# Roco-scientist/NGS-Barcode-Count

Hardware: AMD Instinct MI355X
Metric: reads/sec (whole node), 3x8nt DEL vs 3x1k refs (higher is better)
Workload: dtype u8

## Files before the change

ngs-barcode-count_amd/csrc/bc_device_plan.h:

```cpp
#pragma once
#include "bc_intrin.h"

#ifdef BC_JIT_TU
extern "C" __constant__ uint64_t bc_jit_addr[];
#define BC_ADDR(field, k) bc_jit_addr[index * kAddrPerGroup + (k)]
#define BC_PLAN_ADDR(field, k) bc_jit_addr[kMaxGroups * kAddrPerGroup + (k)]
#define BC_ADDR_COLD(field, k) (*reinterpret_cast<const volatile uint64_t*>(&bc_jit_addr[index * kAddrPerGroup + (k)]))
#else
#define BC_ADDR_COLD(field, k) field
#define BC_ADDR(field, k) field
#define BC_PLAN_ADDR(field, k) field
#endif

namespace bc {

constexpr int kMaxGroups = 18;
constexpr int kAddrPerGroup = 17;
constexpr int kPlanAddrs = 1;
constexpr int kMaxEntries = 160;
constexpr int kMaxRuns = 40;
constexpr int kClasses = 5;
constexpr int kMaxNW = 10;
constexpr uint32_t kFail = 0xFFFFFFFFu;
constexpr uint32_t kDeferred = 0xFFFFFFFEu;
// ... 134 lines not shown
BC_HD uint64_t wide_fingerprint(const uint64_t* key, uint32_t W) {
  uint64_t h = 0x9E3779B97F4A7C15ull;
#pragma unroll
  for (uint32_t w = 1; w < (uint32_t)kMaxKeyWords; ++w)
    if (w < W) h = wide_mix(h ^ key[w]) + w;
  return h >> 1;
}
BC_HD void wide_or_bits(uint64_t (&key)[kMaxKeyWords], uint32_t at, uint32_t v, uint32_t n) {
  const uint32_t w0 = 1u + (at >> 6), sh = at & 63u;
  const uint64_t x = (uint64_t)(v & lowmask(n));
  const bool spill = sh + n > 64u;
  const uint64_t lo = x << sh, hi = spill ? x >> ((64u - sh) & 63u) : 0ull;
#pragma unroll
  for (uint32_t w = 1; w < (uint32_t)kMaxKeyWords; ++w) {
    if (w == w0) key[w] |= lo;
    if (w == w0 + 1u) key[w] |= hi;
  }
}
BC_HD void wide_or_planes(uint64_t (&key)[kMaxKeyWords], uint32_t at, uint32_t q1, uint32_t q2, uint32_t qn, uint32_t len) {
  wide_or_bits(key, at, q1 & ~qn, len);
  wide_or_bits(key, at + len, q2 & ~qn, len);
  wide_or_bits(key, at + 2u * len, qn, len);
}

constexpr int kNCounters = 8;
constexpr int kTotalReads = 6;

enum Outcome : uint32_t {
  kMatched = 0, kConstantRegion = 1, kSampleBarcode = 2, kBarcode = 3, kDuplicate = 4, kLowQuality = 5,
  kPending = 6,
  kUnsupported = 7
};

}
```

ngs-barcode-count_amd/csrc/bc_engine.hip:

```cpp
#include <hip/hip_runtime.h>
#include <string.h>
#include <stdio.h>
#include <stdlib.h>
#include <unistd.h>

#include <algorithm>
#include <functional>
#include <thread>
#include <unordered_map>
#include <string>
#include <vector>

#include "../../include/barcode_count_hip.h"
#include "bc_kernel.h"
#include "bc_engine_impl.h"
#include "bc_fold.h"
#include "bc_synth.h"

extern "C" int bc_internal_table_pack_u8(const void* d_table_u32, const void* d_bits, uint64_t n, void* d_out_u8, void* d_ovf_idx_u64,
                                         void* d_ovf_val_u32, uint64_t ovf_capacity, uint64_t* n_ovf, int device_id, void* hip_stream);

namespace bc {

template <int NW, int NWW>
// ... 614 lines not shown
      if (G.seed_nb) {
        if ((rc = upload(e, H.seed_off.data(), H.seed_off.size() * 4, &G.seed_off_a))) return rc;
        if ((rc = upload(e, H.seed_list.data(), H.seed_list.size() * 4, &G.seed_list_a))) return rc;
        if ((rc = upload(e, H.odd_list.data(), H.odd_list.size() * 4, &G.odd_list_a))) return rc;
        if (G.seed2_nb) {
          if ((rc = upload(e, H.seed2_off.data(), H.seed2_off.size() * 4, &G.seed2_off_a))) return rc;
          if ((rc = upload(e, H.seed2_list.data(), H.seed2_list.size() * 4, &G.seed2_list_a))) return rc;
        }
        if (G.seed3_nb) {
          if ((rc = upload(e, H.seed3_off.data(), H.seed3_off.size() * 4, &G.seed3_off_a))) return rc;
          if ((rc = upload(e, H.seed3_list.data(), H.seed3_list.size() * 4, &G.seed3_list_a))) return rc;
        }
        if (G.tier_blen) {
          if ((rc = upload(e, H.tier_off.data(), H.tier_off.size() * 4, &G.tier_off_a))) return rc;
          if ((rc = upload(e, H.tier_list.data(), H.tier_list.size() * 4, &G.tier_list_a))) return rc;
          if ((rc = upload(e, H.tier_bkt.data(), H.tier_bkt.size() * 4, &G.tier_bkt_a))) return rc;
        }
      }
    }
    if (G.mode == kSetDirect) {
      void* d = nullptr;
      HIP_TRY(hipMalloc(&d, (size_t)4 << (2 * G.len)));
      e->allocs.push_back(d);
      G.dtable_a = (uint64_t)(uintptr_t)d;
    }
  }
  if (const char* cl = getenv("BC_COUNT_LOG")) e->count_log = strcmp(cl, "auto") == 0 ? 2 : atoi(cl);
  if (const char* ch = getenv("BC_COUNT_LOG_HOT")) e->log_hot = atoi(ch) != 0;
  if (const char* cd = getenv("BC_COUNT_LOG_DEFER_RESET")) e->defer_reset = atoi(cd) != 0;
  if (const char* cf = getenv("BC_COUNT_LOG_FRESH")) e->fold_fresh = atoi(cf) != 0;
  if (const char* cm = getenv("BC_COUNT_LOG_MIN_READS")) e->log_min_reads = strtoull(cm, nullptr, 0);
  if (const char* cc = getenv("BC_COUNT_LOG_CHUNK")) {
    const uint64_t c = strtoull(cc, nullptr, 0) & ~63ull;
    if (c) e->log_chunk = std::min<uint64_t>(c, 1ull << 27);
  }
  if (P.lhash_vec) {
    const int rc = upload(e, e->h.lhash.data(), e->h.lhash.size() * 4, &P.lhash_a);
    if (rc) return rc;
  }
#ifdef BC_EXPERIMENT
  if (const char* pm = getenv("BC_PIPE")) e->pipe = atoi(pm) != 0;
#endif
  e->qshare = qual_region_shared();
  HIP_TRY(hipMalloc((void**)&e->d_plan, sizeof(DevPlan)));
  HIP_TRY(hipMemcpy(e->d_plan, &P, sizeof(DevPlan), hipMemcpyHostToDevice));
  for (uint32_t g = 0; g < P.n_groups; ++g) {
    const DevGroup& G = P.groups[g];
    if (G.mode != kSetDirect) continue;
    const uint32_t nq = 1u << (2 * G.len);
    hipLaunchKernelGGL(build_dtable_kernel, dim3((nq + 255) / 256), dim3(256), 0, e->stream, e->d_plan, g,
                       reinterpret_cast<uint32_t*>((uintptr_t)G.dtable_a));
    HIP_TRY(hipGetLastError());
  }
  if (P.sparse) {
    if (table_mem) {
      set_error("bc_engine_create: the plan keeps raw captures (no dense table); pass table_mem = NULL");
      return BC_ERR_INVALID;
    }
  } else if (table_mem) {
    e->d_table = (uint32_t*)table_mem;
    e->table_all_dirty = true;
  } else {
    HIP_TRY(hipMalloc((void**)&e->d_table, e->table_entries * 4));
    e->own_table = true;
    HIP_TRY(hipMemsetAsync(e->d_table, 0, e->table_entries * 4, e->stream));
  }
  if (e->n_bit_words) {
// ... 157 lines not shown
  const OwedPlan owed = owed_plan(e, use_log, table_untouched);
  if (owed.table == kOwedMain) {
    const int rc = settle_table_on(e, e->stream);
    if (rc != BC_OK) return rc;
  }
  if (owed.bits == kOwedMain) {
    const int rc = settle_bits_on(e, e->stream);
    if (rc != BC_OK) return rc;
  }
  const uint32_t flags = (s.pipe ? 1u : 0u) | (s.tables_generic ? 2u : 0u) | (s.hot_generic && hot_on ? 4u : 0u);
  if (s.lds + 64 > e->lds_limit) {
    set_error("read stride too large for one LDS tile");
    return BC_ERR_UNSUPPORTED;
  }
  const bool wide = e->h.plan.wide != 0;
  const void* kern = wide ? (const void*)match_count_wide_kernel<NW, NWW> : (const void*)match_count_kernel<NW, NWW>;
  if (s.lds > 48 * 1024) HIP_TRY(hipFuncSetAttribute(kern, hipFuncAttributeMaxDynamicSharedMemorySize, (int)s.lds));
  int per_cu = 0;
  HIP_TRY(hipOccupancyMaxActiveBlocksPerMultiprocessor(&per_cu, kern, kTPB, lds));
  if (per_cu < 1) per_cu = 1;
  const uint64_t resident = (uint64_t)per_cu * e->n_cus;
  const uint64_t blocks = std::min<uint64_t>((n_reads + kTPB - 1) / kTPB, resident);
  uint64_t blocks_jit = blocks, resident_jit = resident;
  hipEvent_t e0 = nullptr, e1 = nullptr;
  if (e->timing) {
    HIP_TRY(hipEventCreate(&e0));
    HIP_TRY(hipEventCreate(&e1));
    HIP_TRY(hipEventRecord(e0, e->stream));
  }
  hipFunction_t jit_fn = nullptr;
  e->reads_seen += n_reads;
  if (NW <= 8 && NWW <= 4 && e->jit_mode != 0) {
    int per_cu_jit = 1;
    jit_fn = e->jit.function(e->h.plan, e->device, e->jit_mode, e->reads_seen, s, hot_on, &per_cu_jit);
    resident_jit = (uint64_t)per_cu_jit * e->n_cus;
    if (jit_fn) blocks_jit = std::min<uint64_t>((n_reads + kTPB - 1) / kTPB, resident_jit);
  }
  if (use_log) {
    const int rc = ensure_log(e, std::min<uint64_t>(n_reads, e->log_chunk));
    if (rc != BC_OK) return rc;
  }
  const uint64_t chunk = use_log ? e->log_chunk : n_reads;
  bool join = false;
  if (use_log) {
    const int rc = fork_owed(e, owed, &join);
    if (rc != BC_OK) {
      if (join) (void)hipStreamWaitEvent(e->stream, e->reset_join, 0);
      (void)settle_owed(e);
      return rc;
    }
  }
  struct JoinGuard {
    bc_engine* e;
    bool* join;
    ~JoinGuard() {
      if (*join) (void)hipStreamWaitEvent(e->stream, e->reset_join, 0);
    }
  } join_guard{e, &join};
  for (uint64_t c0 = 0; c0 < n_reads; c0 += chunk) {
    const uint64_t n_c = std::min<uint64_t>(chunk, n_reads - c0);
    const uint8_t* a_seq = (const uint8_t*)d_seq + c0 * stride;
    const uint8_t* a_qual = d_qual ? (const uint8_t*)d_qual + c0 * stride : nullptr;
    const uint16_t* a_lens = d_lens ? (const uint16_t*)d_lens + c0 : nullptr;
    const uint16_t* a_qlens = d_qlens ? (const uint16_t*)d_qlens + c0 : nullptr;
    uint8_t* a_to = e->trace_outcome ? e->trace_outcome + trace_off + c0 : nullptr;
    uint64_t* a_ti = e->trace_idx ? e->trace_idx + trace_off + c0 : nullptr;
    uint32_t* a_log = use_log ? e->d_log : nullptr;
// ... 1549 lines not shown
```

ngs-barcode-count_amd/csrc/bc_engine_impl.h:

```cpp
#ifndef BC_ENGINE_IMPL_H
#define BC_ENGINE_IMPL_H

#include <hip/hip_runtime.h>
#include <stdint.h>

#include <string>
#include <utility>
#include <vector>

#include "../../include/barcode_count_hip.h"
#include "bc_enrich.h"
#include "bc_jit.h"
#include "bc_plan.hpp"

#define HIP_TRY(expr)                                                                      \
  do {                                                                                     \
    hipError_t _e = (expr);                                                                \
    if (_e != hipSuccess) {                                                                \
      bc::set_error(std::string(#expr) + ": " + hipGetErrorString(_e));                    \
      if (_e == hipErrorOutOfMemory) (void)hipGetLastError();  \
      return _e == hipErrorOutOfMemory ? BC_ERR_NOMEM : BC_ERR_HIP;                        \
    }                                                                                      \
  } while (0)

struct ScratchGuard {
  std::vector<void*> dev, pinned;
  std::vector<hipEvent_t> events;
  ~ScratchGuard() {
    for (void* p : dev) (void)hipFree(p);
    for (void* p : pinned) (void)hipHostFree(p);
    for (hipEvent_t ev : events) (void)hipEventDestroy(ev);
  }
  template <typename T>
  hipError_t dmalloc(T** out, size_t bytes) {
    void* p = nullptr;
    const hipError_t rc = hipMalloc(&p, bytes ? bytes : 16);
    if (rc == hipSuccess) dev.push_back(p);
    *out = (T*)p;
    return rc;
  }
  template <typename T>
  hipError_t hmalloc(T** out, size_t bytes) {
    void* p = nullptr;
    const hipError_t rc = hipHostMalloc(&p, bytes ? bytes : 16, hipHostMallocDefault);
    if (rc == hipSuccess) pinned.push_back(p);
    *out = (T*)p;
    return rc;
  }
  hipError_t event(hipEvent_t* out) {
    const hipError_t rc = hipEventCreateWithFlags(out, hipEventDisableTiming);
    if (rc == hipSuccess) events.push_back(*out);
    return rc;
  }
};

struct bc_engine {
  int device = 0;
  hipStream_t stream = nullptr;
  bool own_stream = false;
  hipStream_t copy_stream = nullptr;
  bc::HostDevPlan h;
  bc::DevPlan* d_plan = nullptr;
  std::vector<void*> allocs;
  uint32_t* d_table = nullptr;
  bool own_table = false;
  uint64_t table_entries = 0;
  uint32_t* d_bits = nullptr;
  uint64_t n_bit_words = 0;
  bool bits_dirty = false;
  bool table_exposed = false;
  uint64_t dirty_bytes = 0;
  bool table_all_dirty = false;
  uint64_t reads_since_fold = 0;
  int count_log = 2;
  uint64_t log_min_reads = 1ull << 24;
  uint64_t log_chunk = 1ull << 27;
  bool log_hot = false;
  uint64_t log_cap = 0;
  uint32_t* d_log = nullptr;
  uint32_t* d_grouped = nullptr;
  uint64_t gz_segments = 0;
  uint64_t gz_blocks = 0;
  uint64_t log_folds = 0;
  uint32_t* d_fold_meta = nullptr;
  bool owed_table = false;
  bool owed_table_all = false;
  bool owed_bits = false;
  bool defer_reset = true;
  bool fold_fresh = true;
  hipStream_t reset_stream = nullptr;
  hipEvent_t reset_fork = nullptr, reset_join = nullptr;
  unsigned long long* d_counters = nullptr;
  uint32_t barcode_num = 0;
  uint32_t n_sets[bc::kMaxGroups] = {0};
  std::vector<std::vector<std::string>> set_seqs;
  bool has_sample_group = false;
  uint8_t* trace_outcome = nullptr;
  uint64_t* trace_idx = nullptr;
  bool timing = false;
  std::vector<std::pair<hipEvent_t, hipEvent_t>> events;
  std::vector<float> launch_ms;
  std::vector<uint64_t> row_idx;
  std::vector<uint32_t> row_cnt;
  static constexpr int kStages = 2;
  uint8_t* pin[kStages] = {nullptr, nullptr};
  uint8_t* dev[kStages] = {nullptr, nullptr};
  hipEvent_t copied[kStages] = {nullptr, nullptr};
  hipEvent_t consumed[kStages] = {nullptr, nullptr};
  size_t stage_bytes = 0;
// ... 68 lines not shown
```

ngs-barcode-count_amd/csrc/bc_jit.h:

```cpp
#pragma once
#include <hip/hip_runtime.h>
#include <stdint.h>

#include <atomic>
#include <map>
#include <memory>
#include <string>
#include <thread>
#include <vector>

#include "bc_plan.hpp"

namespace bc {

struct PlanSetup {
  int lhash_mode = 1;
  uint64_t n_bit_words = 0;
  uint64_t dirty_bytes = 0;
};
PlanSetup plan_setup(HostDevPlan& h, bool long_only, bool own_table);

inline int generic_nw(uint32_t maxlen) { return maxlen <= 128 ? 4 : (maxlen <= 256 ? 8 : 10); }

struct JitShape {
  int NW, NWW;
  bool lens, tables, trace;
  bool qshare = false;
  uint32_t stride, read_len, region;
  bool conservative = false;
  int min_waves = 3;
};

struct MatchShape {
  int generic_nw;
  uint32_t region;
  uint32_t lds, lds_jit;
  uint32_t lds_cold, lds_jit_cold;
  bool tables_generic, tables_jit;
  bool hot_generic, hot_jit;
  bool pipe;
  JitShape jit;
  int first_min_waves;
  uint64_t key;
};
MatchShape match_shape(const DevPlan& P, uint64_t table_entries, uint32_t stride, uint32_t read_len, bool lens, bool trace,
                       uint32_t lds_limit, bool pipe, bool qshare, int lhash_mode);
bool qual_region_shared();

struct JitKernels {
  struct Jit {
    enum { kIdle = 0, kCompiling = 1, kCodeReady = 2, kLoaded = 3, kFailed = -1 };
    std::atomic<int> state{kIdle};
    std::thread worker;
    std::vector<char> code;
    std::string log;
    hipModule_t mod = nullptr;
    hipFunction_t fn = nullptr;
    int per_cu = 0, per_cu_cold = 0;
  };
  std::map<uint64_t, std::unique_ptr<Jit>> slots;

  JitKernels() = default;
  JitKernels(const JitKernels&) = delete;
  JitKernels& operator=(const JitKernels&) = delete;
  ~JitKernels();
  hipFunction_t function(const DevPlan& plan, int device, int mode, uint64_t reads_seen, const MatchShape& s, bool hot_on,
                         int* per_cu);
};

}
```

ngs-barcode-count_amd/csrc/bc_jit.hip:

```cpp
#include <hip/hip_runtime.h>
#include <hip/hiprtc.h>
#include <dlfcn.h>
#include <errno.h>
#include <fcntl.h>
#include <spawn.h>
#include <stdio.h>
#include <stdlib.h>
#include <string.h>
#include <sys/stat.h>
#include <sys/wait.h>
#include <unistd.h>

#include <algorithm>

#include "../../include/barcode_count_hip.h"
#include "bc_jit.h"
#include "bc_kernel.h"

#include "bc_jit_sources.inc"

extern char** environ;

namespace bc {

// ... 142 lines not shown
  return s;
}

static int code_scratch_bytes(const std::vector<char>& code) {
  static const char kKey[] = ".private_segment_fixed_size";
  const size_t kl = sizeof(kKey) - 1;
  if (code.size() < kl + 5) return -1;
  for (size_t i = 0; i + kl + 5 <= code.size(); ++i) {
    if (code[i] != '.' || memcmp(&code[i], kKey, kl) != 0) continue;
    const unsigned char* v = reinterpret_cast<const unsigned char*>(&code[i + kl]);
    if (v[0] < 0x80) return v[0];
    if (v[0] == 0xcc) return v[1];
    if (v[0] == 0xcd) return (v[1] << 8) | v[2];
    if (v[0] == 0xce) return (int)(((uint32_t)v[1] << 24) | (v[2] << 16) | (v[3] << 8) | v[4]);
    return -1;
  }
  return -1;
}

static void push_flags(std::vector<std::string>& d, const char* flags) {
  std::string t;
  for (const char* c = flags;; ++c) {
    if (*c == ' ' || *c == ';' || *c == 0) {
      if (!t.empty()) d.push_back(t);
      t.clear();
      if (*c == 0) break;
    } else {
      t += *c;
    }
  }
}

static std::vector<std::string> jit_defines(int NW, int NWW, bool lens, bool tables, bool qshare, bool trace, uint32_t stride,
                                            uint32_t read_len, uint32_t region, bool conservative, int min_waves) {
  std::vector<std::string> d = {"-DJIT_NW=" + std::to_string(NW), "-DJIT_NWW=" + std::to_string(NWW),
                                "-DJIT_STRIDE=" + std::to_string(stride), "-DJIT_READ_LEN=" + std::to_string(lens ? 0u : read_len),
                                "-DJIT_REGION=" + std::to_string(region),
                                lens ? "-DJIT_LENS=1" : "-DJIT_LENS=0", tables ? "-DJIT_LHASH=1" : "-DJIT_LHASH=0", qshare ? "-DJIT_QSHARE=1" : "-DJIT_QSHARE=0", trace ? "-DJIT_TRACE=1" : "-DJIT_TRACE=0",
                                "-DBC_MIN_WAVES=" + std::to_string(min_waves), "-DBC_TPB=" + std::to_string(kTPB)};
#ifdef BC_PROFILE
  d.push_back("-DBC_PROFILE=1");
#endif
  if (conservative) d.push_back("-DBC_NO_STATIC_COUNT=1");
#ifdef BC_VARIANT_FLAGS
  push_flags(d, BC_VARIANT_FLAGS);
#endif
#ifdef BC_EXPERIMENT
  d.push_back("-DBC_EXPERIMENT=1");
  if (const char* extra = getenv("BC_JIT_FLAGS")) push_flags(d, extra);
#endif
  return d;
}

static uint64_t fnv1a(const std::string& s, uint64_t h = 0xcbf29ce484222325ull) {
  for (unsigned char c : s) h = (h ^ c) * 0x100000001b3ull;
  return h;
}

static bool read_file(const std::string& path, std::vector<char>& out) {
  FILE* f = fopen(path.c_str(), "rb");
  if (!f) return false;
  fseek(f, 0, SEEK_END);
  const long n = ftell(f);
  fseek(f, 0, SEEK_SET);
  out.resize(n > 0 ? (size_t)n : 0);
  const bool ok = n > 0 && fread(out.data(), 1, (size_t)n, f) == (size_t)n;
  fclose(f);
  return ok;
}

static bool write_file(const std::string& path, const void* data, size_t n) {
  const std::string tmp = path + ".tmp" + std::to_string((long)getpid());
// ... 59 lines not shown
  std::vector<char*> argv;
  for (auto& a : argv_s) argv.push_back(const_cast<char*>(a.c_str()));
  argv.push_back(nullptr);
  posix_spawn_file_actions_t fa;
  posix_spawn_file_actions_init(&fa);
  posix_spawn_file_actions_addopen(&fa, 1, err.c_str(), O_WRONLY | O_CREAT | O_TRUNC, 0644);
  posix_spawn_file_actions_adddup2(&fa, 1, 2);
  std::vector<char*> envp;
  for (char** ev = environ; ev && *ev; ++ev) {
    static const char* const kDrop[] = {"LD_PRELOAD=", "ROCP", "ROCPROF", "HSA_TOOLS", "ROCTX", "BC_", "HIP_LAUNCH_BLOCKING="};
    bool drop = false;
    for (const char* d : kDrop) drop = drop || strncmp(*ev, d, strlen(d)) == 0;
    if (!drop) envp.push_back(*ev);
  }
  envp.push_back(nullptr);
  pid_t pid = 0;
  int rc = posix_spawn(&pid, driver.c_str(), &fa, nullptr, argv.data(), envp.data());
  posix_spawn_file_actions_destroy(&fa);
  if (rc == 0) {
    int status = 0;
    while (waitpid(pid, &status, 0) < 0 && errno == EINTR) {
    }
    rc = (WIFEXITED(status) && WEXITSTATUS(status) == 0) ? 0 : 1;
  }
  std::vector<char> lg;
  if (read_file(err, lg)) log.assign(lg.begin(), lg.end());
  const bool ok = rc == 0 && read_file(out, code);
  remove(out.c_str());
  remove(err.c_str());
  if (ok) remove(in.c_str());
  return ok;
}

static bool jit_get_code(const DevPlan& P, const std::string& arch, const JitShape& sh, bool may_compile,
                         const char* store_dir, std::vector<char>& code, std::string& log) {
  const std::string src = jit_source(P);
  const std::vector<std::string> defs = jit_defines(sh.NW, sh.NWW, sh.lens, sh.tables, sh.qshare, sh.trace, sh.stride, sh.read_len, sh.region, sh.conservative, sh.min_waves);
  std::string key = arch + "\n" + src;
  for (const auto& d : defs) key += d;
  for (int i = 0; i < kJitHdrs; ++i) key += kJitHdrText[i];
  char name[64];
  snprintf(name, sizeof name, "bcjit_%016llx", (unsigned long long)fnv1a(key));
  if (const char* src_out = getenv("BC_JIT_SRC")) write_file(src_out, src.data(), src.size());
  std::vector<std::string> dirs;
  if (store_dir) dirs.push_back(store_dir);
  if (const char* c = getenv("BC_JIT_CACHE")) dirs.push_back(c);
  dirs.push_back(lib_cache_dir());
  const char* drv = getenv("BC_JIT_COMPILER");
  const std::string driver = drv ? drv : "/opt/rocm/bin/hipcc";
  const bool have_driver = driver != "rtc" && access(driver.c_str(), X_OK) == 0;
  for (const auto& d : dirs)
    if (!d.empty() && read_file(d + "/" + name + ".co", code)) return true;
  if (!have_driver)
    for (const auto& d : dirs)
      if (!d.empty() && read_file(d + "/" + name + "_rtc.co", code)) return true;
  if (!may_compile) {
    log = "not in the kernel cache";
    return false;
  }
  std::string wdir;
  for (const auto& d : dirs) {
    if (d.empty()) continue;
    mkdir(d.c_str(), 0755);
    if (access(d.c_str(), W_OK) == 0) {
      wdir = d;
      break;
    }
  }
  if (wdir.empty()) {
    const char* t = getenv("TMPDIR");
    wdir = std::string(t && *t ? t : "/tmp") + "/barcode-count-jit-" + std::to_string((long)getuid());
    mkdir(wdir.c_str(), 0700);
    if (access(wdir.c_str(), W_OK) != 0) wdir.clear();
  }
  bool ok = false, by_driver = false;
  if (have_driver && !wdir.empty()) ok = by_driver = jit_compile_driver(driver, wdir, name, src, arch, defs, code, log);
  if (!ok) ok = jit_compile_rtc(src, arch, defs, code, log);
  if (ok && !wdir.empty()) write_file(wdir + "/" + name + (by_driver ? ".co" : "_rtc.co"), code.data(), code.size());
  return ok;
}

static bool jit_pick_code(const DevPlan& P, const std::string& arch, JitShape sh, int first_mw, bool may_compile,
                          const char* store_dir, std::vector<char>& code, std::string& log) {
  const int floor_mw = std::min(first_mw, sh.NW > 4 ? 2 : 3);
  for (int pass = 0; pass < 2; ++pass) {
    sh.conservative = pass == 1;
    for (int mw = pass == 0 ? first_mw : floor_mw; mw >= (pass == 0 ? floor_mw : 2); --mw) {
      sh.min_waves = mw;
      if (!jit_get_code(P, arch, sh, may_compile, store_dir, code, log)) return false;
      const int scratch = code_scratch_bytes(code);
      if (scratch == 0) return true;
#ifdef BC_EXPERIMENT
      if (getenv("BC_JIT_ALLOW_SCRATCH")) return true;
#endif
      log = "the build for " + std::to_string(mw) + " waves per SIMD needs " + std::to_string(scratch) + " bytes of scratch memory per lane";
    }
  }
  code.clear();
  return false;
}

static std::string jit_arch(int device) {
  hipDeviceProp_t prop;
  std::string arch = "gfx950";
  if (hipGetDeviceProperties(&prop, device) == hipSuccess && prop.gcnArchName[0]) arch = prop.gcnArchName;
  const size_t colon = arch.find(':');
  if (colon != std::string::npos) arch.resize(colon);
  return arch;
}

static bool jit_load(const DevPlan& plan, JitKernels::Jit& out) {
  if (const char* dump = getenv("BC_JIT_DUMP")) write_file(dump, out.code.data(), out.code.size());
  hipDeviceptr_t addr = nullptr;
  size_t addr_bytes = 0;
  if (hipModuleLoadData(&out.mod, out.code.data()) != hipSuccess ||
      hipModuleGetFunction(&out.fn, out.mod, "bc_jit_match_count") != hipSuccess ||
      hipModuleGetGlobal(&addr, &addr_bytes, out.mod, "bc_jit_addr") != hipSuccess ||
      addr_bytes != (kMaxGroups * kAddrPerGroup + kPlanAddrs) * sizeof(uint64_t)) {
    fprintf(stderr, "[barcode-count] scheme-specialised kernel did not load; using the generic kernel\n");
    out.fn = nullptr;
    return false;
  }
  int scratch = 0;
  bool allow_scratch = false;
#ifdef BC_EXPERIMENT
  allow_scratch = getenv("BC_JIT_ALLOW_SCRATCH") != nullptr;
#endif
  if (hipFuncGetAttribute(&scratch, HIP_FUNC_ATTRIBUTE_LOCAL_SIZE_BYTES, out.fn) == hipSuccess && scratch > 0 && !allow_scratch) {
    fprintf(stderr, "[barcode-count] scheme-specialised kernel build uses %d bytes of scratch memory per lane: not used\n", scratch);
    (void)hipModuleUnload(out.mod);
    out.mod = nullptr;
    out.fn = nullptr;
    return false;
  }
  std::vector<uint64_t> table(kMaxGroups * kAddrPerGroup + kPlanAddrs, 0);
  for (int g = 0; g < kMaxGroups; ++g) {
    uint64_t* f[kAddrPerGroup];
    DevGroup G = plan.groups[g];
    addr_fields(G, f);
    for (int k = 0; k < kAddrPerGroup; ++k) table[g * kAddrPerGroup + k] = *f[k];
  }
  table[kMaxGroups * kAddrPerGroup] = plan.lhash_a;
  if (hipMemcpyHtoD(addr, table.data(), table.size() * sizeof(uint64_t)) != hipSuccess) {
    out.fn = nullptr;
    return false;
  }
  std::vector<char>().swap(out.code);
  return true;
}

hipFunction_t JitKernels::function(const DevPlan& plan, int device, int mode, uint64_t reads_seen, const MatchShape& s,
                                   bool hot_on, int* per_cu) {
  const JitShape& sh = s.jit;
  const int first_mw = s.first_min_waves;
  auto& slot = slots[s.key];
  if (!slot) slot.reset(new Jit());
  Jit& j = *slot;
  typedef Jit J;
  if (j.state.load(std::memory_order_acquire) == J::kIdle) {
    const std::string arch = jit_arch(device);
    if (jit_pick_code(plan, arch, sh, first_mw, false, nullptr, j.code, j.log)) {
      j.state.store(J::kCodeReady, std::memory_order_release);
    } else if (mode == 2) {
      const bool ok = jit_pick_code(plan, arch, sh, first_mw, true, nullptr, j.code, j.log);
      if (!ok)
        fprintf(stderr, "[barcode-count] scheme-specialised kernel did not compile; using the generic kernel\n%.2000s\n",
                j.log.c_str());
      j.state.store(ok ? J::kCodeReady : J::kFailed, std::memory_order_release);
    } else if (mode == 1) {
      if (reads_seen < (1ull << 20)) return nullptr;
      j.state.store(J::kCompiling, std::memory_order_release);
      const DevPlan own = plan;
      Jit* jp = &j;
      const JitShape shape = sh;
      j.worker = std::thread([jp, own, arch, shape, first_mw]() {
        const bool ok = jit_pick_code(own, arch, shape, first_mw, true, nullptr, jp->code, jp->log);
        jp->state.store(ok ? J::kCodeReady : J::kFailed, std::memory_order_release);
      });
    } else {
      j.state.store(J::kFailed, std::memory_order_release);
    }
  }
  if (j.state.load(std::memory_order_acquire) == J::kCodeReady) {
    if (j.worker.joinable()) j.worker.join();
    bool ok = jit_load(plan, j);
    if (!ok) fprintf(stderr, "[barcode-count] using the generic kernel\n");
    if (ok && (hipModuleOccupancyMaxActiveBlocksPerMultiprocessor(&j.per_cu, j.fn, kTPB, s.lds_jit) != hipSuccess || j.per_cu < 1))
      j.per_cu = 1;
    if (ok && (hipModuleOccupancyMaxActiveBlocksPerMultiprocessor(&j.per_cu_cold, j.fn, kTPB, s.lds_jit_cold) != hipSuccess ||
               j.per_cu_cold < 1))
      j.per_cu_cold = 1;
    j.state.store(ok ? J::kLoaded : J::kFailed, std::memory_order_release);
  }
  if (j.state.load(std::memory_order_acquire) == J::kFailed && j.worker.joinable()) {
    j.worker.join();
    fprintf(stderr, "[barcode-count] scheme-specialised kernel did not compile; using the generic kernel\n%.2000s\n",
            j.log.c_str());
  }
  if (j.state.load(std::memory_order_acquire) != J::kLoaded) return nullptr;
  *per_cu = hot_on ? j.per_cu : j.per_cu_cold;
  return j.fn;
}

JitKernels::~JitKernels() {
  for (auto& kv : slots) {
    if (kv.second->worker.joinable()) kv.second->worker.join();
    if (kv.second->mod) (void)hipModuleUnload(kv.second->mod);
  }
}

}

using namespace bc;

extern "C" int bc_internal_jit_compile(const bc_plan* p, uint32_t stride, uint32_t read_len, int lens, const char* cache_dir,
                                       const char* out_path) {
  if (!p) {
    set_error("bc_plan_precompile: null plan");
    return BC_ERR_INVALID;
  }
  HostDevPlan h;
  const char* wl_env = getenv("BC_WIDE_LANE");
  if (!p->lower(h, wl_env && atoi(wl_env) != 0)) return BC_ERR_UNSUPPORTED;
  const PlanSetup ps = plan_setup(h, false, true);
  const uint32_t maxlen = lens ? stride : read_len;
  if (maxlen == 0 || maxlen > stride || maxlen > 256) {
    set_error("bc_plan_precompile: read_len must be in 1..stride and at most 256 bases for a specialised kernel");
    return BC_ERR_INVALID;
  }
  bool pipe = true;
#ifdef BC_EXPERIMENT
  if (const char* pm = getenv("BC_PIPE")) pipe = atoi(pm) != 0;
#endif
  const MatchShape s = match_shape(h.plan, h.plan.sparse ? 0 : h.table_entries, stride, read_len, lens != 0, false,
                                   kGfx950LdsBytes, pipe, qual_region_shared(), ps.lhash_mode);
  std::vector<char> code;
  std::string log;
  const std::string dir = cache_dir ? cache_dir : lib_cache_dir();
  if (!jit_pick_code(h.plan, "gfx950", s.jit, s.first_min_waves, true, dir.c_str(), code, log)) {
    set_error("scheme-specialised kernel did not compile: " + log);
    return BC_ERR_INVALID;
  }
  if (out_path) write_file(out_path, code.data(), code.size());
  return BC_OK;
}

extern "C" int bc_internal_match_shape(const bc_plan* p, uint32_t stride, uint32_t read_len, int lens, int qshare, uint64_t* key,
                                       uint32_t* lds_hot, uint32_t* lds_cold, uint32_t* region, uint32_t* tables_bytes,
                                       int* shared) {
  HostDevPlan h;
  if (!p || !p->lower(h)) return BC_ERR_UNSUPPORTED;
  const PlanSetup ps = plan_setup(h, false, true);
  const MatchShape s = match_shape(h.plan, h.plan.sparse ? 0 : h.table_entries, stride, read_len, lens != 0, true,
                                   kGfx950LdsBytes, true, qshare != 0, ps.lhash_mode);
  *key = s.key;
  *lds_hot = s.lds_jit;
  *lds_cold = s.lds_jit_cold;
  *region = s.region;
  *tables_bytes = s.tables_jit ? h.plan.lhash_vec * 16u : 0u;
  *shared = s.jit.qshare ? 1 : 0;
  return BC_OK;
}

int bc_plan_precompile(const bc_plan* p, uint32_t stride, uint32_t read_len, int with_lens, const char* cache_dir) {
  return bc_internal_jit_compile(p, stride, read_len, with_lens, cache_dir, nullptr);
}
```

ngs-barcode-count_amd/csrc/bc_kernel.h:

```cpp
#pragma once
#include "bc_lane.h"
#include "bc_long.h"

#ifdef BC_PROFILE
extern "C" __device__ unsigned long long bc_g_profile[16];
#endif

namespace bc {

#ifndef BC_TPB
#define BC_TPB 256
#endif
constexpr int kTPB = BC_TPB;
#ifndef BC_MIN_WAVES
#define BC_MIN_WAVES 3
#endif

__device__ __forceinline__ uint32_t lane_now() {
  uint32_t l;
  asm volatile("v_mbcnt_lo_u32_b32 %0, -1, 0\n\tv_mbcnt_hi_u32_b32 %0, -1, %0" : "=v"(l));
  return l;
}
__device__ __forceinline__ uint32_t wave_min_u32(uint32_t v) {
#pragma unroll
  for (int o = 32; o > 0; o >>= 1) {
    const uint32_t t = (uint32_t)__shfl_xor((int)v, o);
    v = t < v ? t : v;
  }
  return v;
}

__device__ __forceinline__ uint32_t wave_verdict(const Nearest& s, uint32_t max_err) {
  const uint32_t kmin = wave_min_u32(s.key);
  const unsigned long long holders = __ballot(s.key == kmin);
  const int first = __ffsll(holders) - 1;
  const uint32_t cnt = (uint32_t)__shfl((int)s.count, first);
  const uint32_t idx = (uint32_t)__shfl((int)s.idx, first);
  const bool unique = __popcll(holders) == 1 && kmin != 0xFFFFFFFFu;
  return unique ? nearest_result(kmin, idx, cnt, max_err) : kFail;
}

__device__ __forceinline__ uint32_t wave_fix_error(const DevGroup& G, uint32_t q1, uint32_t q2, uint32_t qn, uint32_t qx,
                                                   bool use_exact) {
  const uint32_t lane = lane_now();
  Nearest s;
  nearest_init(s);
// ... 640 lines not shown
    if (abl_ & 0x100000u) todo &= ~probed;
    while (todo) {
      const int src = __ffsll(todo) - 1;
      todo &= todo - 1;
      const uint32_t b1 = (uint32_t)__shfl((int)q1, src);
      const uint32_t b2 = (uint32_t)__shfl((int)q2, src);
      const uint32_t bn = (uint32_t)__shfl((int)qn, src);
      const uint32_t bx = (uint32_t)__shfl((int)qx, src);
      const bool seeded = !defer_ && G.seed_nb && bx == 0u && G.n_odd == 0u && __popc(bn) <= 2;
      const uint32_t r = seeded ? wave_fix_error_seeded(G, b1, b2, bn, ((probed >> src) & 1ull) != 0ull)
                                : wave_fix_error(G, b1, b2, bn, bx, true);
      if (lane == (uint32_t)src) out = r;
    }
    return out;
  }
};

template <int NW, int NWW, bool kLens, bool kAligned = false, bool kWide = false>
__device__ __forceinline__ void match_count_body(const DevPlan& pl, const uint8_t* __restrict__ seq,
                                                 const uint8_t* __restrict__ qual, const uint16_t* __restrict__ lens,
                                                 const uint16_t* __restrict__ qlens,
                                                 uint32_t stride, uint32_t read_len, uint32_t nd, uint64_t n_reads,
                                                 uint32_t region, uint32_t* __restrict__ table, uint32_t* __restrict__ bits,
                                                 unsigned long long* __restrict__ slots, uint32_t* __restrict__ vals,
                                                 uint64_t smask, unsigned long long* __restrict__ counters,
                                                 uint8_t* __restrict__ trace_outcome, uint64_t* __restrict__ trace_idx,
                                                 uint32_t flags, uint32_t* __restrict__ count_log = nullptr,
                                                 uint32_t* __restrict__ ready = nullptr) {
  extern __shared__ uint4 smem[];
  __shared__ uint32_t s_cnt[kNCounters];
  const uint32_t tid = threadIdx.x;
  const uint32_t lane = tid & 63u;
  const bool queues = pl.defer_search();
  const uint32_t wave = queues ? (uint32_t)__builtin_amdgcn_readfirstlane((int)(tid >> 6)) : tid >> 6;
  if (tid < kNCounters) s_cnt[tid] = 0;

  const bool with_qual = pl.quality_on && !(pl.abl() & 0x8u);
  const bool pipe = (flags & 1u) != 0u;
#ifdef JIT_LHASH
  const uint32_t lhash_vec = JIT_LHASH ? pl.lhash_vec : 0u;
#else
  const uint32_t lhash_vec = (flags & 2u) ? pl.lhash_vec : 0u;
#endif
  DeviceOps ops;
  {
    Quad* area = reinterpret_cast<Quad*>(smem);
    const BC_GLOBAL Quad* image = reinterpret_cast<const BC_GLOBAL Quad*>(pl.lhash_image());
    for (uint32_t i = tid; i < lhash_vec; i += kTPB) area[i] = image[i];
    ops.area = area;
    ops.with_tables = lhash_vec != 0u;
    ops.abl_ = pl.abl();
  }
  const bool hot = (flags & 4u) != 0u;
  const uint32_t hot_seed = blockIdx.x * 0x85EBCA6Bu;
  uint32_t* hot_tag = reinterpret_cast<uint32_t*>(reinterpret_cast<uint8_t*>(smem) + lhash_vec * 16u);
  uint32_t* hot_cnt = hot_tag + kHotSlots;
  if (hot) {
    for (uint32_t i = tid; i < kHotSlots; i += kTPB) {
      hot_tag[i] = kHotEmpty;
      hot_cnt[i] = 0u;
    }
  }
#ifdef JIT_QSHARE
  const bool share = JIT_QSHARE != 0 && with_qual;
#else
  const bool share = false;
#endif
  const uint32_t two = (with_qual && pipe && !share) ? 2u : 1u;
  ops.defer_ = queues && !(pl.abl() & 0x200000u);
  uint4* const dq = reinterpret_cast<uint4*>(reinterpret_cast<uint8_t*>(smem) + lhash_vec * 16u + (hot ? kHotBytes : 0u) + wave * kQueueBytes);
  uint32_t dq_plain = 0, dq_n = 0;
  uint32_t tile_seq = 0;
  ops.tile = reinterpret_cast<uint8_t*>(smem) + lhash_vec * 16u + (hot ? kHotBytes : 0u) + (queues ? (kTPB / 64) * kQueueBytes : 0u) +
             wave * region * two;
  ops.qtile = ops.tile + (two == 2u ? region : 0u);
  ops.share = share;
  ops.region = region;
  ops.lane = lane;
  ops.stride_ = stride;
  const uint32_t full_bytes = 64u * stride;
  ops.chunks = (full_bytes + 1023u) / 1024u;
  ops.pending_add = 0;

  const uint64_t n_tiles = (n_reads + 63u) >> 6;
  const uint64_t n_full = n_reads >> 6;
  const uint64_t n_waves = (uint64_t)gridDim.x * (kTPB / 64);
  uint32_t acc_cnt[kNCounters];
#pragma unroll
  for (int k = 0; k < kNCounters; ++k) acc_cnt[k] = 0;
  for (uint32_t i = full_bytes + lane; i < region; i += 64) {
    ops.tile[i] = 'A';
    if (with_qual && !share) ops.qtile[i] = 'I';
  }
  const bool logm = count_log != nullptr;
  uint32_t first_old = 0, first_on = 0, direct_tiles = 0;
  uint64_t first_idx = 0;
  uint64_t t = (uint64_t)blockIdx.x * (kTPB / 64) + wave;
  bool seq_ready = false, qual_ready = false;
  if (t < n_full && pipe) {
    dma_tile(ops.tile, seq + (t << 6) * stride, full_bytes, lane);
    seq_ready = true;
    if (with_qual && !share) {
      dma_tile(ops.qtile, qual + (t << 6) * stride, full_bytes, lane);
      qual_ready = true;
    }
  }
  __syncthreads();
#ifdef BC_PROFILE
  for (int k = 0; k < 12; ++k) ops.acc[k] = 0;
  ops.t_last = __builtin_readcyclecounter();
#endif
  auto hot_count = [&](bool add, uint32_t key) -> bool {
    uint32_t h = ((key ^ hot_seed) * 0x9E3779B1u) >> (32u - kHotBits);
    uint32_t tag = add ? hot_tag[h] : key ^ 1u;
#ifndef BC_HOT_ONE
    if (add && tag != key && tag != kHotEmpty) {
      h = ((key ^ hot_seed) * 0xC2B2AE35u) >> (32u - kHotBits);
      tag = hot_tag[h];
    }
#endif
    if (add && tag == kHotEmpty) {
      const uint32_t old = atomicCAS(&hot_tag[h], kHotEmpty, key);
      tag = old == kHotEmpty ? key : old;
    }
    if (add && tag == key) {
      atomicAdd(&hot_cnt[h], 1u);
      add = false;
    }
    return add;
  };
  for (; t < n_tiles; t += n_waves) {
    const uint64_t wfirst = t << 6;
    const uint32_t n_w = n_reads - wfirst < 64u ? (uint32_t)(n_reads - wfirst) : 64u;
    const uint64_t goff = wfirst * stride;
    const uint64_t tn = t + n_waves;
    const bool next_full = tn < n_full && pipe;
    ops.qsrc = qual + goff;
    ops.bytes = n_w * stride;
    ops.next_seq = next_full ? seq + (tn << 6) * stride : nullptr;
    ops.qual_async = share ? seq_ready : qual_ready;
    if (seq_ready) {
      wait_vm_keep((qual_ready ? ops.chunks : 0u) + ops.pending_add);
      wave_lds_fence();
    } else {
      wave_lds_fence();
      stage_tile(ops.tile, seq + goff, ops.bytes, full_bytes, (uint8_t)'A', lane);
      wave_lds_fence();
    }

    ops.mark(1);
    const bool active = lane < n_w;
    uint32_t len = 0;
    if (active) len = kLens ? (uint32_t)lens[wfirst + lane] : read_len;
    uint32_t qlen = len;
    if (kLens && qlens && active) qlen = (uint32_t)qlens[wfirst + lane];
    const uint32_t base = (active ? lane : 0u) * stride;
    const ReadResultT<kWide> r = process_read<DeviceOps, NW, NWW, kAligned, kWide>(
        pl, ops, reinterpret_cast<const uint32_t*>(ops.tile), base, len, qlen, nd, active);

    ops.mark(8);
    uint32_t outcome = r.outcome;
    uint64_t wide_slot = 0;
    if constexpr (kWide) {
      const bool ins = active && outcome == kMatched && (pl.has_random || !pl.discard_counts);
      if (__any(ins)) {
        bool is_new;
        wide_slot = wide_insert_lanes(slots, ready, smask, pl.key_words, r.wkey, ins, is_new);
        if (pl.has_random && ins && !is_new) outcome = kDuplicate;
      }
    } else if (pl.has_random) {
      if (active && outcome == kMatched && !set_insert(slots, smask, r.dense_idx * pl.rspace + r.rcode))
        outcome = kDuplicate;
    }
#pragma unroll
    for (uint32_t k = 0; k < kNCounters; ++k) {
      if (k == kTotalReads) continue;
      acc_cnt[k] += (uint32_t)__popcll(__ballot(active && outcome == k));
    }
    acc_cnt[kTotalReads] += n_w;
    if (trace_outcome && active && !(queues && outcome == kPending)) {
      trace_outcome[wfirst + lane] = (uint8_t)outcome;
      if constexpr (kWide)
        trace_idx[wfirst + lane] = (outcome == kMatched || outcome == kDuplicate) ? r.wkey[0] : 0ull;
      else
        trace_idx[wfirst + lane] = pl.has_random ? r.dense_idx * pl.rspace + r.rcode : r.dense_idx;
    }
    bool repeat = false;
    if (bits && !logm) repeat = first_on != 0u && ((first_old >> ((uint32_t)first_idx & 31u)) & 1u) != 0u;
    const uint64_t repeat_idx = first_idx;
    seq_ready = next_full;
    qual_ready = false;
    if (next_full && with_qual && !share) {
      wave_lds_fence();
      dma_tile(ops.qtile, qual + (tn << 6) * stride, full_bytes, lane);
      qual_ready = true;
    }
    ops.pending_add = 0;
    if (bits && !logm) {
      const uint32_t n_rep = (uint32_t)__popcll(__ballot(repeat));
      if (n_rep) {
        if (repeat) table_add_marked(pl, table, bits, repeat_idx);
        ops.pending_add += 1u;
        if (2u * n_rep > (uint32_t)__popcll(__ballot(first_on != 0u))) direct_tiles = 16u;
      }
      if (direct_tiles) --direct_tiles;
    }
    first_on = 0u;
    if constexpr (kWide) {
      if (!pl.has_random && active && outcome == kMatched && !pl.discard_counts) atomicAdd(&vals[wide_slot], 1u);
    } else if (!pl.has_random) {
      bool add = active && outcome == kMatched && !pl.discard_counts && !(pl.abl() & 0x4u);
      if (hot && !pl.sparse && __any(add)) add = hot_count(add, (uint32_t)r.dense_idx);
      if (logm) {
        if (active) count_log[wfirst + lane] = add ? (uint32_t)r.dense_idx : kLogNone;
        ops.pending_add += 1u;
      } else if (__any(add)) {
        if (add) {
          if (pl.sparse) {
            atomicAdd(&vals[map_slot(slots, smask, r.dense_idx)], 1u);
          } else if (bits && direct_tiles == 0u) {
            first_old = atomicOr(&bits[r.dense_idx >> 5], 1u << ((uint32_t)r.dense_idx & 31u));
            first_idx = r.dense_idx;
            first_on = 1u;
          } else {
            table_add_marked(pl, table, bits, r.dense_idx);
          }
        }
// ... 47 lines not shown
          uint32_t res;
          if (!coarse_with_n(G, b1, b2, bn, res)) res = (pl.abl() & 0x100000u) ? kFail : wave_fix_error_seeded(G, b1, b2, bn, true);
          settle(lane == 0u, res, where);
        }
        while (dq_plain >= ((tn < n_tiles && !pendm) ? 4u : 1u)) {
          const uint32_t n_seg = dq_plain < 4u ? dq_plain : 4u;
          dq_plain -= n_seg;
          const uint32_t seg = lane >> 4;
          const bool seg_on = seg < n_seg;
          const uint4 q = dq[dq_plain + (seg_on ? seg : 0u)];
          CoarseVote vote;
          coarse_probe_x4(G, q.x, q.y, seg_on, vote);
          uint32_t res = kFail;
#pragma unroll
          for (int k = 0; k < 4; ++k) {
            if ((uint32_t)k >= n_seg) break;
            uint32_t kmin, idx, rk;
            bool uniq;
            coarse_segment(vote, k, kmin, uniq, idx);
            if (kmin != 0xFFFFFFFFu && kmin <= G.seed2_nb)
              rk = (uniq && (kmin == 0u || kmin - 1u <= G.max_err)) ? idx : kFail;
            else if (pl.abl() & 0x100000u)
              rk = kFail;
            else
              rk = wave_fix_error_seeded(G, rdlane(q.x, 16 * k), rdlane(q.y, 16 * k), 0u, true);
            res = (int)lane == 16 * k ? rk : res;
          }
          settle(seg_on && (lane & 15u) == 0u, res, q.w);
        }
        if (!pendm) break;
      }
      ++tile_seq;
    }
  }
  if (bits && first_on != 0u && ((first_old >> ((uint32_t)first_idx & 31u)) & 1u) != 0u) table_add_marked(pl, table, bits, first_idx);
#ifdef BC_PROFILE
  if (lane == 0)
    for (int k = 0; k < 12; ++k) atomicAdd(&bc_g_profile[k], ops.acc[k]);
#endif

  if (lane == 0) {
#pragma unroll
    for (uint32_t k = 0; k < kNCounters; ++k)
      if (acc_cnt[k]) atomicAdd(&s_cnt[k], acc_cnt[k]);
  }
  __syncthreads();
  if (tid < kNCounters) {
    const uint32_t v = s_cnt[tid];
    if (v) atomicAdd(&counters[tid], (unsigned long long)v);
  }
  if (hot) {
    for (uint32_t i = tid; i < kHotSlots; i += kTPB) {
      const uint32_t c = hot_cnt[i];
      if (c) {
        atomicAdd(&table[hot_tag[i]], c);
        if (bits && pl.dirty_off) reinterpret_cast<uint8_t*>(bits + pl.dirty_off)[hot_tag[i] >> 6] = (uint8_t)1;
      }
    }
  }
}

}
```

Baseline: 20.38 billion.

## Specialise JIT kernel for count-log mode with 32-bit tiles and packed outcome counters

Adds a JIT variant keyed on count-log and hot-table mode, so the kernel knows at compile time that log mode is on and whether the hot table is used. In that variant tile indices are 32-bit, the tile loop is split into a full-tile pipelined pass and a tail pass with constant seq/qual readiness, and the wave index is made uniform. Per-read outcome counts are packed into a 64-bit byte-lane accumulator and reduced with shuffles every 255 tiles instead of seven ballots per tile. The aim is less scalar and vector work per tile and lower register pressure, at the cost of compiling and caching extra kernel variants.

Result: faster. 21.53 billion (median of 6 runs) (+5.6%).

```diff
diff --git a/ngs-barcode-count_amd/csrc/bc_device_plan.h b/ngs-barcode-count_amd/csrc/bc_device_plan.h
--- a/ngs-barcode-count_amd/csrc/bc_device_plan.h
+++ b/ngs-barcode-count_amd/csrc/bc_device_plan.h
@@ -190,4 +190,23 @@
   kUnsupported = 7
 };
 
-}
+constexpr uint32_t kPackTiles = 255u;
+BC_HD uint64_t outcome_pack(bool active, uint32_t outcome) { return (uint64_t)(active ? 1u : 0u) << (8u * outcome); }
+BC_HD void outcome_split(uint64_t pk, uint32_t (&w)[4]) {
+  const uint32_t lo = (uint32_t)pk, hi = (uint32_t)(pk >> 32);
+  w[0] = lo & 0x00FF00FFu;
+  w[1] = (lo >> 8) & 0x00FF00FFu;
+  w[2] = hi & 0x00FF00FFu;
+  w[3] = (hi >> 8) & 0x00FF00FFu;
+}
+BC_HD void outcome_fold(const uint32_t (&sums)[4], uint32_t (&acc)[kNCounters]) {
+  acc[0] += sums[0] & 0xFFFFu;
+  acc[2] += sums[0] >> 16;
+  acc[1] += sums[1] & 0xFFFFu;
+  acc[3] += sums[1] >> 16;
+  acc[4] += sums[2] & 0xFFFFu;
+  acc[5] += sums[3] & 0xFFFFu;
+  acc[7] += sums[3] >> 16;
+}
+
+}
diff --git a/ngs-barcode-count_amd/csrc/bc_engine.hip b/ngs-barcode-count_amd/csrc/bc_engine.hip
--- a/ngs-barcode-count_amd/csrc/bc_engine.hip
+++ b/ngs-barcode-count_amd/csrc/bc_engine.hip
@@ -670,7 +670,8 @@
   if (const char* cm = getenv("BC_COUNT_LOG_MIN_READS")) e->log_min_reads = strtoull(cm, nullptr, 0);
   if (const char* cc = getenv("BC_COUNT_LOG_CHUNK")) {
     const uint64_t c = strtoull(cc, nullptr, 0) & ~63ull;
-    if (c) e->log_chunk = std::min<uint64_t>(c, 1ull << 27);
+    static_assert(kLogChunkMax <= (1ull << 37), "tile_t: tile number + waves of the grid must not wrap");
+    if (c) e->log_chunk = std::min<uint64_t>(c, kLogChunkMax);
   }
   if (P.lhash_vec) {
     const int rc = upload(e, e->h.lhash.data(), e->h.lhash.size() * 4, &P.lhash_a);
@@ -894,7 +895,7 @@
   e->reads_seen += n_reads;
   if (NW <= 8 && NWW <= 4 && e->jit_mode != 0) {
     int per_cu_jit = 1;
-    jit_fn = e->jit.function(e->h.plan, e->device, e->jit_mode, e->reads_seen, s, hot_on, &per_cu_jit);
+    jit_fn = e->jit.function(e->h.plan, e->device, e->jit_mode, e->reads_seen, s, jit_variant(s, use_log, hot_on), &per_cu_jit);
     resident_jit = (uint64_t)per_cu_jit * e->n_cus;
     if (jit_fn) blocks_jit = std::min<uint64_t>((n_reads + kTPB - 1) / kTPB, resident_jit);
   }
diff --git a/ngs-barcode-count_amd/csrc/bc_engine_impl.h b/ngs-barcode-count_amd/csrc/bc_engine_impl.h
--- a/ngs-barcode-count_amd/csrc/bc_engine_impl.h
+++ b/ngs-barcode-count_amd/csrc/bc_engine_impl.h
@@ -54,6 +54,8 @@
   }
 };
 
+constexpr uint64_t kLogChunkMax = 1ull << 27;
+
 struct bc_engine {
   int device = 0;
   hipStream_t stream = nullptr;
@@ -74,7 +76,7 @@
   uint64_t reads_since_fold = 0;
   int count_log = 2;
   uint64_t log_min_reads = 1ull << 24;
-  uint64_t log_chunk = 1ull << 27;
+  uint64_t log_chunk = kLogChunkMax;
   bool log_hot = false;
   uint64_t log_cap = 0;
   uint32_t* d_log = nullptr;
diff --git a/ngs-barcode-count_amd/csrc/bc_jit.h b/ngs-barcode-count_amd/csrc/bc_jit.h
--- a/ngs-barcode-count_amd/csrc/bc_jit.h
+++ b/ngs-barcode-count_amd/csrc/bc_jit.h
@@ -31,6 +31,13 @@
   int min_waves = 3;
 };
 
+struct JitVariant {
+  int count;
+  bool hot;
+  uint32_t id() const { return count == 1 ? (hot ? 3u : 2u) : 0u;  }
+};
+inline JitVariant jit_variant(const struct MatchShape& s, bool use_log, bool hot_on);
+
 struct MatchShape {
   int generic_nw;
   uint32_t region;
@@ -46,6 +53,9 @@
 MatchShape match_shape(const DevPlan& P, uint64_t table_entries, uint32_t stride, uint32_t read_len, bool lens, bool trace,
                        uint32_t lds_limit, bool pipe, bool qshare, int lhash_mode);
 bool qual_region_shared();
+inline JitVariant jit_variant(const MatchShape& s, bool use_log, bool hot_on) {
+  return JitVariant{use_log ? 1 : 2, s.hot_jit && hot_on};
+}
 
 struct JitKernels {
   struct Jit {
@@ -58,13 +68,13 @@
     hipFunction_t fn = nullptr;
     int per_cu = 0, per_cu_cold = 0;
   };
-  std::map<uint64_t, std::unique_ptr<Jit>> slots;
+  std::map<std::pair<uint64_t, uint32_t>, std::unique_ptr<Jit>> slots;
 
   JitKernels() = default;
   JitKernels(const JitKernels&) = delete;
   JitKernels& operator=(const JitKernels&) = delete;
   ~JitKernels();
-  hipFunction_t function(const DevPlan& plan, int device, int mode, uint64_t reads_seen, const MatchShape& s, bool hot_on,
+  hipFunction_t function(const DevPlan& plan, int device, int mode, uint64_t reads_seen, const MatchShape& s, const JitVariant& v,
                          int* per_cu);
 };
 
diff --git a/ngs-barcode-count_amd/csrc/bc_jit.hip b/ngs-barcode-count_amd/csrc/bc_jit.hip
--- a/ngs-barcode-count_amd/csrc/bc_jit.hip
+++ b/ngs-barcode-count_amd/csrc/bc_jit.hip
@@ -198,12 +198,17 @@
 }
 
 static std::vector<std::string> jit_defines(int NW, int NWW, bool lens, bool tables, bool qshare, bool trace, uint32_t stride,
-                                            uint32_t read_len, uint32_t region, bool conservative, int min_waves) {
+                                            uint32_t read_len, uint32_t region, bool conservative, int min_waves,
+                                            const JitVariant& v) {
   std::vector<std::string> d = {"-DJIT_NW=" + std::to_string(NW), "-DJIT_NWW=" + std::to_string(NWW),
                                 "-DJIT_STRIDE=" + std::to_string(stride), "-DJIT_READ_LEN=" + std::to_string(lens ? 0u : read_len),
                                 "-DJIT_REGION=" + std::to_string(region),
                                 lens ? "-DJIT_LENS=1" : "-DJIT_LENS=0", tables ? "-DJIT_LHASH=1" : "-DJIT_LHASH=0", qshare ? "-DJIT_QSHARE=1" : "-DJIT_QSHARE=0", trace ? "-DJIT_TRACE=1" : "-DJIT_TRACE=0",
                                 "-DBC_MIN_WAVES=" + std::to_string(min_waves), "-DBC_TPB=" + std::to_string(kTPB)};
+  if (v.count == 1) {
+    d.push_back("-DJIT_COUNT=1");
+    d.push_back(v.hot ? "-DJIT_HOT=1" : "-DJIT_HOT=0");
+  }
 #ifdef BC_PROFILE
   d.push_back("-DBC_PROFILE=1");
 #endif
@@ -329,10 +334,10 @@
   return ok;
 }
 
-static bool jit_get_code(const DevPlan& P, const std::string& arch, const JitShape& sh, bool may_compile,
+static bool jit_get_code(const DevPlan& P, const std::string& arch, const JitShape& sh, const JitVariant& v, bool may_compile,
                          const char* store_dir, std::vector<char>& code, std::string& log) {
   const std::string src = jit_source(P);
-  const std::vector<std::string> defs = jit_defines(sh.NW, sh.NWW, sh.lens, sh.tables, sh.qshare, sh.trace, sh.stride, sh.read_len, sh.region, sh.conservative, sh.min_waves);
+  const std::vector<std::string> defs = jit_defines(sh.NW, sh.NWW, sh.lens, sh.tables, sh.qshare, sh.trace, sh.stride, sh.read_len, sh.region, sh.conservative, sh.min_waves, v);
   std::string key = arch + "\n" + src;
   for (const auto& d : defs) key += d;
   for (int i = 0; i < kJitHdrs; ++i) key += kJitHdrText[i];
@@ -377,14 +382,14 @@
   return ok;
 }
 
-static bool jit_pick_code(const DevPlan& P, const std::string& arch, JitShape sh, int first_mw, bool may_compile,
+static bool jit_pick_code(const DevPlan& P, const std::string& arch, JitShape sh, const JitVariant& v, int first_mw, bool may_compile,
                           const char* store_dir, std::vector<char>& code, std::string& log) {
   const int floor_mw = std::min(first_mw, sh.NW > 4 ? 2 : 3);
   for (int pass = 0; pass < 2; ++pass) {
     sh.conservative = pass == 1;
     for (int mw = pass == 0 ? first_mw : floor_mw; mw >= (pass == 0 ? floor_mw : 2); --mw) {
       sh.min_waves = mw;
-      if (!jit_get_code(P, arch, sh, may_compile, store_dir, code, log)) return false;
+      if (!jit_get_code(P, arch, sh, v, may_compile, store_dir, code, log)) return false;
       const int scratch = code_scratch_bytes(code);
       if (scratch == 0) return true;
 #ifdef BC_EXPERIMENT
@@ -447,19 +452,19 @@
 }
 
 hipFunction_t JitKernels::function(const DevPlan& plan, int device, int mode, uint64_t reads_seen, const MatchShape& s,
-                                   bool hot_on, int* per_cu) {
+                                   const JitVariant& v, int* per_cu) {
   const JitShape& sh = s.jit;
   const int first_mw = s.first_min_waves;
-  auto& slot = slots[s.key];
+  auto& slot = slots[std::make_pair(s.key, v.id())];
   if (!slot) slot.reset(new Jit());
   Jit& j = *slot;
   typedef Jit J;
   if (j.state.load(std::memory_order_acquire) == J::kIdle) {
     const std::string arch = jit_arch(device);
-    if (jit_pick_code(plan, arch, sh, first_mw, false, nullptr, j.code, j.log)) {
+    if (jit_pick_code(plan, arch, sh, v, first_mw, false, nullptr, j.code, j.log)) {
       j.state.store(J::kCodeReady, std::memory_order_release);
     } else if (mode == 2) {
-      const bool ok = jit_pick_code(plan, arch, sh, first_mw, true, nullptr, j.code, j.log);
+      const bool ok = jit_pick_code(plan, arch, sh, v, first_mw, true, nullptr, j.code, j.log);
       if (!ok)
         fprintf(stderr, "[barcode-count] scheme-specialised kernel did not compile; using the generic kernel\n%.2000s\n",
                 j.log.c_str());
@@ -470,8 +475,9 @@
       const DevPlan own = plan;
       Jit* jp = &j;
       const JitShape shape = sh;
-      j.worker = std::thread([jp, own, arch, shape, first_mw]() {
-        const bool ok = jit_pick_code(own, arch, shape, first_mw, true, nullptr, jp->code, jp->log);
+      const JitVariant var = v;
+      j.worker = std::thread([jp, own, arch, shape, var, first_mw]() {
+        const bool ok = jit_pick_code(own, arch, shape, var, first_mw, true, nullptr, jp->code, jp->log);
         jp->state.store(ok ? J::kCodeReady : J::kFailed, std::memory_order_release);
       });
     } else {
@@ -495,7 +501,7 @@
             j.log.c_str());
   }
   if (j.state.load(std::memory_order_acquire) != J::kLoaded) return nullptr;
-  *per_cu = hot_on ? j.per_cu : j.per_cu_cold;
+  *per_cu = v.hot ? j.per_cu : j.per_cu_cold;
   return j.fn;
 }
 
@@ -531,14 +537,23 @@
 #endif
   const MatchShape s = match_shape(h.plan, h.plan.sparse ? 0 : h.table_entries, stride, read_len, lens != 0, false,
                                    kGfx950LdsBytes, pipe, qual_region_shared(), ps.lhash_mode);
-  std::vector<char> code;
-  std::string log;
+  int count_log = 2;
+  if (const char* cl = getenv("BC_COUNT_LOG")) count_log = strcmp(cl, "auto") == 0 ? 2 : atoi(cl);
+  const char* lh = getenv("BC_COUNT_LOG_HOT");
+  const bool log_hot = lh && atoi(lh) != 0;
+  const bool can_log = count_log != 0 && ps.n_bit_words != 0 && !h.plan.discard_counts && h.table_entries != 0 &&
+                       h.table_entries < 0xFFFFFFFFull;
   const std::string dir = cache_dir ? cache_dir : lib_cache_dir();
-  if (!jit_pick_code(h.plan, "gfx950", s.jit, s.first_min_waves, true, dir.c_str(), code, log)) {
-    set_error("scheme-specialised kernel did not compile: " + log);
-    return BC_ERR_INVALID;
-  }
-  if (out_path) write_file(out_path, code.data(), code.size());
+  for (int use_log = 0; use_log <= (can_log ? 1 : 0); ++use_log) {
+    std::vector<char> code;
+    std::string log;
+    const JitVariant v = jit_variant(s, use_log != 0, use_log ? log_hot : true);
+    if (!jit_pick_code(h.plan, "gfx950", s.jit, v, s.first_min_waves, true, dir.c_str(), code, log)) {
+      set_error("scheme-specialised kernel did not compile: " + log);
+      return BC_ERR_INVALID;
+    }
+    if (out_path && use_log == (can_log ? 1 : 0)) write_file(out_path, code.data(), code.size());
+  }
   return BC_OK;
 }
 
diff --git a/ngs-barcode-count_amd/csrc/bc_kernel.h b/ngs-barcode-count_amd/csrc/bc_kernel.h
--- a/ngs-barcode-count_amd/csrc/bc_kernel.h
+++ b/ngs-barcode-count_amd/csrc/bc_kernel.h
@@ -12,6 +12,24 @@
 #define BC_TPB 256
 #endif
 constexpr int kTPB = BC_TPB;
+#ifndef JIT_COUNT
+#define JIT_COUNT 0
+#endif
+#ifndef JIT_HOT
+#define JIT_HOT (-1)
+#endif
+#if defined(BC_JIT_TU) && JIT_COUNT == 1
+#define BC_LOG_LOOP 1
+#endif
+#ifdef BC_LOG_LOOP
+typedef uint32_t tile_t;
+#else
+typedef uint64_t tile_t;
+#endif
+template <int K>
+struct TileKind {
+  static constexpr int value = K;
+};
 #ifndef BC_MIN_WAVES
 #define BC_MIN_WAVES 3
 #endif
@@ -718,7 +736,11 @@
   const uint32_t tid = threadIdx.x;
   const uint32_t lane = tid & 63u;
   const bool queues = pl.defer_search();
+#ifdef BC_LOG_LOOP
+  const uint32_t wave = (uint32_t)__builtin_amdgcn_readfirstlane((int)(tid >> 6));
+#else
   const uint32_t wave = queues ? (uint32_t)__builtin_amdgcn_readfirstlane((int)(tid >> 6)) : tid >> 6;
+#endif
   if (tid < kNCounters) s_cnt[tid] = 0;
 
   const bool with_qual = pl.quality_on && !(pl.abl() & 0x8u);
@@ -737,7 +759,7 @@
     ops.with_tables = lhash_vec != 0u;
     ops.abl_ = pl.abl();
   }
-  const bool hot = (flags & 4u) != 0u;
+  const bool hot = JIT_HOT >= 0 ? JIT_HOT != 0 : (flags & 4u) != 0u;
   const uint32_t hot_seed = blockIdx.x * 0x85EBCA6Bu;
   uint32_t* hot_tag = reinterpret_cast<uint32_t*>(reinterpret_cast<uint8_t*>(smem) + lhash_vec * 16u);
   uint32_t* hot_cnt = hot_tag + kHotSlots;
@@ -768,26 +790,37 @@
   ops.chunks = (full_bytes + 1023u) / 1024u;
   ops.pending_add = 0;
 
-  const uint64_t n_tiles = (n_reads + 63u) >> 6;
-  const uint64_t n_full = n_reads >> 6;
-  const uint64_t n_waves = (uint64_t)gridDim.x * (kTPB / 64);
+  const tile_t n_tiles = (tile_t)((n_reads + 63u) >> 6);
+  const tile_t n_full = (tile_t)(n_reads >> 6);
+  const tile_t n_waves = (tile_t)gridDim.x * (kTPB / 64);
+  auto tile_off = [&](tile_t x) -> uint64_t {
+#ifdef BC_LOG_LOOP
+    return (uint64_t)x * full_bytes;
+#else
+    return (x << 6) * stride;
+#endif
+  };
   uint32_t acc_cnt[kNCounters];
 #pragma unroll
   for (int k = 0; k < kNCounters; ++k) acc_cnt[k] = 0;
+#ifdef BC_LOG_LOOP
+  uint64_t pk_cnt = 0;
+  uint32_t pk_tiles = 0;
+#endif
   for (uint32_t i = full_bytes + lane; i < region; i += 64) {
     ops.tile[i] = 'A';
     if (with_qual && !share) ops.qtile[i] = 'I';
   }
-  const bool logm = count_log != nullptr;
+  const bool logm = JIT_COUNT == 1 ? true : (JIT_COUNT == 2 ? false : count_log != nullptr);
   uint32_t first_old = 0, first_on = 0, direct_tiles = 0;
   uint64_t first_idx = 0;
-  uint64_t t = (uint64_t)blockIdx.x * (kTPB / 64) + wave;
+  tile_t t = (tile_t)blockIdx.x * (kTPB / 64) + wave;
   bool seq_ready = false, qual_ready = false;
   if (t < n_full && pipe) {
-    dma_tile(ops.tile, seq + (t << 6) * stride, full_bytes, lane);
+    dma_tile(ops.tile, seq + tile_off(t), full_bytes, lane);
     seq_ready = true;
     if (with_qual && !share) {
-      dma_tile(ops.qtile, qual + (t << 6) * stride, full_bytes, lane);
+      dma_tile(ops.qtile, qual + tile_off(t), full_bytes, lane);
       qual_ready = true;
     }
   }
@@ -815,18 +848,30 @@
     }
     return add;
   };
+#ifdef BC_LOG_LOOP
+  auto tile_body = [&](auto kind_c) __attribute__((always_inline)) {
+    constexpr int kKind = decltype(kind_c)::value;
+#else
   for (; t < n_tiles; t += n_waves) {
-    const uint64_t wfirst = t << 6;
+    constexpr int kKind = 0;
+#endif
+    const uint64_t wfirst = (uint64_t)t << 6;
+#ifdef BC_LOG_LOOP
+    const uint32_t n_w = (kKind == 1 || t < n_full) ? 64u : (uint32_t)n_reads & 63u;
+#else
     const uint32_t n_w = n_reads - wfirst < 64u ? (uint32_t)(n_reads - wfirst) : 64u;
-    const uint64_t goff = wfirst * stride;
-    const uint64_t tn = t + n_waves;
+#endif
+    const uint64_t goff = tile_off(t);
+    const tile_t tn = t + n_waves;
     const bool next_full = tn < n_full && pipe;
     ops.qsrc = qual + goff;
     ops.bytes = n_w * stride;
-    ops.next_seq = next_full ? seq + (tn << 6) * stride : nullptr;
-    ops.qual_async = share ? seq_ready : qual_ready;
-    if (seq_ready) {
-      wait_vm_keep((qual_ready ? ops.chunks : 0u) + ops.pending_add);
+    ops.next_seq = next_full ? seq + tile_off(tn) : nullptr;
+    const bool seq_here = kKind == 1 ? true : (kKind == 2 ? false : seq_ready);
+    const bool qual_here = kKind == 1 ? (with_qual && !share) : (kKind == 2 ? false : qual_ready);
+    ops.qual_async = share ? seq_here : qual_here;
+    if (seq_here) {
+      wait_vm_keep((qual_here ? ops.chunks : 0u) + ops.pending_add);
       wave_lds_fence();
     } else {
       wave_lds_fence();
@@ -858,11 +903,26 @@
       if (active && outcome == kMatched && !set_insert(slots, smask, r.dense_idx * pl.rspace + r.rcode))
         outcome = kDuplicate;
     }
+#ifdef BC_LOG_LOOP
+    pk_cnt += outcome_pack(active, outcome);
+    if (++pk_tiles == kPackTiles || tn >= n_tiles) {
+      uint32_t w[4];
+      outcome_split(pk_cnt, w);
+#pragma unroll
+      for (int j = 0; j < 4; ++j)
+#pragma unroll
+        for (int o = 32; o > 0; o >>= 1) w[j] += (uint32_t)__shfl_xor((int)w[j], o);
+      outcome_fold(w, acc_cnt);
+      pk_cnt = 0;
+      pk_tiles = 0;
+    }
+#else
 #pragma unroll
     for (uint32_t k = 0; k < kNCounters; ++k) {
       if (k == kTotalReads) continue;
       acc_cnt[k] += (uint32_t)__popcll(__ballot(active && outcome == k));
     }
+#endif
     acc_cnt[kTotalReads] += n_w;
     if (trace_outcome && active && !(queues && outcome == kPending)) {
       trace_outcome[wfirst + lane] = (uint8_t)outcome;
@@ -878,7 +938,7 @@
     qual_ready = false;
     if (next_full && with_qual && !share) {
       wave_lds_fence();
-      dma_tile(ops.qtile, qual + (tn << 6) * stride, full_bytes, lane);
+      dma_tile(ops.qtile, qual + tile_off(tn), full_bytes, lane);
       qual_ready = true;
     }
     ops.pending_add = 0;
@@ -992,7 +1052,13 @@
       }
       ++tile_seq;
     }
-  }
+#ifndef BC_LOG_LOOP
+  }
+#else
+  };
+  for (const tile_t n_ahead = pipe ? n_full : 0u; t < n_ahead; t += n_waves) tile_body(TileKind<1>{});
+  for (; t < n_tiles; t += n_waves) tile_body(TileKind<2>{});
+#endif
   if (bits && first_on != 0u && ((first_old >> ((uint32_t)first_idx & 31u)) & 1u) != 0u) table_add_marked(pl, table, bits, first_idx);
 #ifdef BC_PROFILE
   if (lane == 0)
```
